# spcl/gemm_hls

Hardware: AMD Instinct MI355X
Metric: GFLOP/s, fp32 GEMM N=K=M=16384 per MI355X (tiled outer-product C=A.B), and % of fp32 MFMA peak (higher is better)
Workload: dtype f32; 1 GPU; float 16384x16384x16384 (Multiply,Add) on 1 MI355X; BASELINE configs[1]; kernel=mfma_f32_256x256x16_w8_flush4096, rows_total=16384, rows_per_gpu=16384

## Files before the change

### gemm_hls_amd/csrc/mm_mfma_f32.hip

```cpp
#include <cstdlib>
#include <type_traits>

#include "mm_common.h"

namespace mm {
namespace {

#include "mm_mfma_f32_tile.inc"
#include "mm_mfma_f32_small.inc"
#include "mm_mfma_f32_streamk.inc"

__global__ __launch_bounds__(256) void splitk_reduce_kernel(const float *__restrict__ partials, float *__restrict__ C,
                                                            size_t quads, unsigned splits) {
  const size_t i = (size_t)blockIdx.x * 256 + threadIdx.x;
  if (i >= quads) return;
  const f32x4 *src = (const f32x4 *)partials;
  f32x4 acc = src[i];
  for (unsigned s = 1; s < splits; ++s) acc += src[(size_t)s * quads + i];
  ((f32x4 *)C)[i] = acc;
}

template <typename G, bool AT = false>
int launch_geo(hipStream_t s, const Problem &p, unsigned splits = 1) {
  const unsigned tiles_n = (p.n + G::BM - 1) / G::BM, tiles_m = (p.m + G::BN - 1) / G::BN;
  static unsigned long long configured = 0;
  if (int e = ensure_dynamic_lds((const void *)mfma_f32_kernel<G, AT>, G::LDS_BYTES, configured)) return e;
  (void)hipGetLastError();
  if (splits <= 1) {
    hipLaunchKernelGGL((mfma_f32_kernel<G, AT>), dim3(tiles_n * tiles_m), dim3(G::THREADS), G::LDS_BYTES, s,
                       (const float *)p.a, (const float *)p.b, (float *)p.c, p.n, p.k, p.m, tiles_n, tiles_m,
                       band_rows(G::BM, G::BN, G::MIN_WAVES), 0u, (float *)nullptr);
    return (int)hipGetLastError();
  }
  const unsigned chunk = ((p.k + splits - 1) / splits + 31u) & ~31u;
  const size_t plane = (size_t)p.n * p.m;
  int dev = 0;
  hipError_t e = hipGetDevice(&dev);
  if (e != hipSuccess) return (int)e;
  hipMemPool_t pool = nullptr;
  if (int rc = workspace_pool(dev, &pool)) return rc;
  float *ws = nullptr;
  if ((e = hipMallocFromPoolAsync((void **)&ws, plane * splits * sizeof(float), pool, s)) != hipSuccess) return (int)e;
  hipLaunchKernelGGL((mfma_f32_kernel<G, AT>), dim3(tiles_n * tiles_m * splits), dim3(G::THREADS), G::LDS_BYTES, s,
                     (const float *)p.a, (const float *)p.b, (float *)p.c, p.n, p.k, p.m, tiles_n, tiles_m,
                     band_rows(G::BM, G::BN, G::MIN_WAVES), chunk, ws);
  int rc = (int)hipGetLastError();
  if (rc == 0) {
    const size_t quads = plane / 4;
    hipLaunchKernelGGL(splitk_reduce_kernel, dim3((unsigned)((quads + 255) / 256)), dim3(256), 0, s, ws, (float *)p.c, quads, splits);
    rc = (int)hipGetLastError();
  }
  const hipError_t f = hipFreeAsync(ws, s);
  return rc ? rc : (int)f;
}

template <typename G, bool AT, bool SEED>
__global__ __launch_bounds__(G::THREADS, G::MIN_WAVES) void mfma_f32_batched_kernel(
    const float *__restrict__ A, const float *__restrict__ B, float *__restrict__ C, unsigned N, unsigned K, unsigned M,
    unsigned tiles_n, unsigned tiles_m, unsigned kBand, unsigned batch, size_t stride_a, size_t stride_b, size_t stride_c) {
  const unsigned lin = batched_tile(A, B, C, tiles_n * tiles_m, batch, stride_a, stride_b, stride_c);
  const unsigned band = lin / (kBand * tiles_m), within = lin % (kBand * tiles_m);
  const unsigned rows_in_band = min(kBand, tiles_n - band * kBand);
  const unsigned tile_row = band * kBand + within % rows_in_band;
  const unsigned tile_col = within / rows_in_band;
  tile_body<G, AT, false, SEED>(A, B, C, N, K, M, K, M, N, M, tile_row * G::BM, tile_col * G::BN);
}

template <typename G, bool AT, bool SEED>
int launch_geo_batched_seed(hipStream_t s, const Problem &p) {
  const unsigned tiles_n = (p.n + G::BM - 1) / G::BM, tiles_m = (p.m + G::BN - 1) / G::BN;
  static unsigned long long configured = 0;
  (void)hipGetLastError();
  if (int e = ensure_dynamic_lds((const void *)mfma_f32_batched_kernel<G, AT, SEED>, G::LDS_BYTES, configured)) return e;
  hipLaunchKernelGGL((mfma_f32_batched_kernel<G, AT, SEED>), dim3(tiles_n * tiles_m * p.batch), dim3(G::THREADS), G::LDS_BYTES,
                     s, (const float *)p.a, (const float *)p.b, (float *)p.c, p.n, p.k, p.m, tiles_n, tiles_m,
                     band_rows(G::BM, G::BN, G::MIN_WAVES), p.batch, p.stride_a, p.stride_b, p.stride_c);
  return (int)hipGetLastError();
}

template <typename G, bool AT = false>
int launch_geo_batched(hipStream_t s, const Problem &p) {
  return p.seed ? launch_geo_batched_seed<G, AT, true>(s, p) : launch_geo_batched_seed<G, AT, false>(s, p);
}

using T128x256 = Geo<2, 2, 2, 16, Chain::FlushIntoC, 256, Reads::Pipelined, Dma::ScalarBase>;
using T128x256v = Geo<2, 2, 2, 16, Chain::FlushIntoC, 256, Reads::Pipelined, Dma::VectorAddress>;
using T256x256 = Geo<2, 4, 2, 16, Chain::FlushIntoC, 256, Reads::Pipelined, Dma::ScalarBase>;
using T256x256v = Geo<2, 4, 2, 16, Chain::FlushIntoC, 256, Reads::Pipelined, Dma::VectorAddress>;
using T128x128 = Geo<1, 4, 1, 32, Chain::FlushIntoC, 128, Reads::Pipelined, Dma::ScalarBase>;
using T128x128v = Geo<1, 4, 1, 32, Chain::FlushIntoC, 128, Reads::Pipelined, Dma::VectorAddress>;
using X128x256x32_2lvl = Geo<2, 2, 2, 32, Chain::TwoLevel, 16, Reads::CompilerPlaced, Dma::VectorAddress>;
using X256x256_single = Geo<2, 4, 2, 16, Chain::Single, 1, Reads::CompilerPlaced, Dma::VectorAddress>;

struct VariantInfo { int id; const char *name; unsigned bm, bn, bk, waves; };
template <typename G> constexpr VariantInfo info_of(int id, const char *name) { return {id, name, G::BM, G::BN, G::BK, G::NW}; }
constexpr VariantInfo kVariants[] = {
    info_of<T128x256>(33, "mfma_f32_128x256x16_w4x2_flush4096"),
    info_of<T256x256>(8, "mfma_f32_256x256x16_w8_flush4096"),
    info_of<T128x128>(35, "mfma_f32_128x128x32_w4x2_flush4096"),
    info_of<Small>(64, "mfma_f32_64x64x32_w4x2_flush4096"),
    info_of<X128x256x32_2lvl>(0, "mfma_f32_128x256x32_w4_2lvl"),
    info_of<X256x256_single>(3, "mfma_f32_256x256x16_w8"),
};

const VariantInfo *find_variant(int v) {
  for (const VariantInfo &i : kVariants)
    if (i.id == v) return &i;
  return nullptr;
}

}

int mfma_f32_num_variants() { return (int)(sizeof(kVariants) / sizeof(kVariants[0])); }
int mfma_f32_variant_id(int index) { return index >= 0 && index < mfma_f32_num_variants() ? kVariants[index].id : -1; }

static const TileCandidate kAutoCands[] = {{33, 128, 256, 2, 1.00}, {8, 256, 256, 1, 0.991}, {35, 128, 128, 2, 0.993}};

static bool streamk_wins(const Problem &p) {
  if (p.a_transposed || p.k % 32 != 0 || p.k < 256 || p.n_total) return false;
  if ((unsigned long long)((p.n + 127) / 128) * ((p.m + 127) / 128) * (p.k / 32) >= (1ull << 31)) return false;
  const double tiles = (double)((p.n + 127) / 128) * ((p.m + 127) / 128);
  const unsigned tn = (p.n + 127) / 128, tm = (p.m + 127) / 128;
  const bool teams_4x4 = tn % 4 == 0 && tm % 4 == 0;
  if (tiles <= 256 || tiles > (teams_4x4 ? 4096 : 2304)) return false;
  double whole = 0;
  pick_tile(kAutoCands, 3, p.n, p.m, &whole);
  const double sk = (2.0 * tiles / 512 + 0.25) * 128 * 128 / 0.993;
  return sk < 0.99 * whole;
}

template <typename G>
static int launch_small(hipStream_t s, const Problem &p, unsigned splits) {
  const unsigned tiles_n = (p.n + G::BM - 1) / G::BM, tiles_m = (p.m + G::BN - 1) / G::BN;
  static unsigned long long configured = 0;
  if (int e = ensure_dynamic_lds((const void *)mfma_f32_small_kernel<G>, G::LDS_BYTES, configured)) return e;
  (void)hipGetLastError();
  const unsigned kband = band_rows(G::BM, G::BN, G::PER_CU);
  if (splits <= 1) {
    hipLaunchKernelGGL((mfma_f32_small_kernel<G>), dim3(tiles_n * tiles_m), dim3(G::THREADS), G::LDS_BYTES, s, (const float *)p.a,
                       (const float *)p.b, (float *)p.c, p.n, p.k, p.m, tiles_n, tiles_m, kband, 0u, (float *)nullptr);
    return (int)hipGetLastError();
  }
  const unsigned chunk = ((p.k + splits - 1) / splits + 31u) & ~31u;
  if ((unsigned long long)(splits - 1) * chunk >= p.k) return kErrNotSupported;
  const size_t plane = (size_t)p.n * p.m;
  int dev = 0;
  hipError_t e = hipGetDevice(&dev);
  if (e != hipSuccess) return (int)e;
  hipMemPool_t pool = nullptr;
  if (int rc = workspace_pool(dev, &pool)) return rc;
  float *ws = nullptr;
  if ((e = hipMallocFromPoolAsync((void **)&ws, plane * splits * sizeof(float), pool, s)) != hipSuccess) return (int)e;
  hipLaunchKernelGGL((mfma_f32_small_kernel<G>), dim3(tiles_n * tiles_m * splits), dim3(G::THREADS), G::LDS_BYTES, s, (const float *)p.a,
                     (const float *)p.b, (float *)p.c, p.n, p.k, p.m, tiles_n, tiles_m, kband, chunk, ws);
  int rc = (int)hipGetLastError();
  if (rc == 0) {
    const size_t quads = plane / 4;
    hipLaunchKernelGGL(splitk_reduce_kernel, dim3((unsigned)((quads + 255) / 256)), dim3(256), 0, s, ws, (float *)p.c, quads, splits);
    rc = (int)hipGetLastError();
  }
  const hipError_t f = hipFreeAsync(ws, s);
  return rc ? rc : (int)f;
}

static unsigned auto_split_chunks(unsigned long long tiles, unsigned k) {
  unsigned s = tiles <= 192 ? (unsigned)(512 / tiles) : 1;
  if (s > 8) s = 8;
  while (s > 1 && k / s < 256) --s;
  return s;
}

static bool small_fits(const Problem &p) {
  return !p.a_transposed && 64ull * p.k * 4ull < (1ull << 32) && 32ull * p.m * 4ull < (1ull << 32);
}

static unsigned small_split_chunks(const Problem &p) {
  const unsigned rows = p.n_total ? p.n_total : p.n;
  const unsigned long long t64 = (unsigned long long)((rows + 63) / 64) * ((p.m + 63) / 64);
  if (tuning(TUNE_F32_SPLITK) == 1 || t64 > 128) return 1;
  unsigned s = (unsigned)(256 / t64);
  if (s > 8) s = 8;
  while (s > 1 && p.k / s < 512) --s;
  const double slabs = (p.k + 31) / 32;
  return (s > 1 && 13.5 + (slabs / s) * 0.52 < slabs * 0.52) ? s : 1;
}
static bool small_wins(const Problem &p) {
  if (!small_fits(p) || p.k < 32) return false;
  const unsigned rows = p.n_total ? p.n_total : p.n;
  const unsigned long long t64 = (unsigned long long)((rows + 63) / 64) * ((p.m + 63) / 64), t128 = (unsigned long long)((rows + 127) / 128) * ((p.m + 127) / 128);
  if (t64 > 512) return false;
  const double slabs = (p.k + 31) / 32;
  const unsigned ss = small_split_chunks(p);
  const double t_small = 3.5 + (ss > 1 ? 13.5 : 0.0) + (slabs / ss) * (t64 * ss <= 256 ? 0.52 : 0.90);
  const unsigned s = tuning(TUNE_F32_SPLITK) == 1 ? 1 : auto_split_chunks(t128, p.k);
  const double t_128 = (s > 1 ? 18.5 : 5.0) + (slabs / s) * (t128 * s <= 256 ? 1.79 : 3.49);
  return t_small < t_128;
}

int mfma_f32_auto_variant(const Problem &p) {
  const int knob = tuning(TUNE_F32_SPLITK);
  if (knob < 0 && streamk_wins(p)) return 35;
  const int v = pick_tile(kAutoCands, 3, p.n, p.m);
  if (v == 35 && (knob < 0 || knob == 1) && small_wins(p)) return 64;
  if (v == 33) {
    const unsigned long long t256 = (unsigned long long)((p.n + 255) / 256) * ((p.m + 255) / 256);
    if (t256 % 256 == 0 && t256 >= 4 * 256) return 8;
  }
  return v;
}

bool mfma_f32_serves(const Problem &p) {
  if (!(p.n >= 1 && p.m >= 4 && p.k >= 8 && p.m % 4 == 0 && p.k % 8 == 0)) return false;
  return !p.a_transposed || (p.n >= 4 && p.n % 4 == 0);
}

static bool transposes_first(const Problem &p, int variant_knob) {
  if (!p.a_transposed || variant_knob >= 0) return false;
  const unsigned long long tiles = (unsigned long long)((p.n + 255) / 256) * ((p.m + 255) / 256), rounds = (tiles + 255) / 256;
  if ((double)tiles >= 0.93 * (double)(rounds * 256)) return false;
  return (unsigned long long)p.n * p.k * sizeof(float) <= (2ull << 30);
}
static Problem as_row_major(const Problem &p) {
  Problem q = p;
  q.a_transposed = false;
  return q;
}

__global__ __launch_bounds__(256) void transpose_kxn_kernel(const float *__restrict__ src, float *__restrict__ dst, unsigned K, unsigned N) {
  __shared__ float tile[64][65];
  const unsigned blocks_n = (N + 63) / 64;
  const unsigned k0 = (blockIdx.x / blocks_n) * 64, n0 = (blockIdx.x % blocks_n) * 64;
#pragma unroll
  for (int i = 0; i < 4; ++i) {
    const unsigned idx = threadIdx.x + 256 * i, r = idx >> 4, c = (idx & 15u) * 4;
    if (k0 + r < K && n0 + c < N) {
      const f32x4 v = *(const f32x4 *)(src + (size_t)(k0 + r) * N + n0 + c);
#pragma unroll
      for (int j = 0; j < 4; ++j) tile[r][c + j] = v[j];
    }
  }
  __syncthreads();
#pragma unroll
  for (int i = 0; i < 4; ++i) {
    const unsigned idx = threadIdx.x + 256 * i, r = idx >> 4, c = (idx & 15u) * 4;
    if (n0 + r < N && k0 + c < K) {
      f32x4 v;
#pragma unroll
      for (int j = 0; j < 4; ++j) v[j] = tile[c + j][r];
      *(f32x4 *)(dst + (size_t)(n0 + r) * K + k0 + c) = v;
    }
  }
}

int mfma_f32_resolve(const Problem &p, int variant) {
  if (!mfma_f32_serves(p)) return -1;
  if (p.a_transposed) {
    if (transposes_first(p, variant)) return mfma_f32_resolve(as_row_major(p), variant);
    return 8;
  }
  if (variant < 0) variant = mfma_f32_auto_variant(p);
  if (variant == 64 && !small_fits(p)) return -1;
  return find_variant(variant) ? variant : -1;
}

int mfma_f32_splitk(const Problem &p, int variant) {
  if (p.a_transposed) return transposes_first(p, tuning(TUNE_F32_VARIANT)) ? mfma_f32_splitk(as_row_major(p), variant) : 1;
  if (variant == 64) {
    const int forced = tuning(TUNE_F32_SPLITK);
    unsigned s = forced >= 2 && forced <= 8 ? (unsigned)forced : tuning(TUNE_F32_VARIANT) >= 0 ? 1u : small_split_chunks(p);
    while (s > 1 && p.k / s < 64) --s;
    return (int)s;
  }
  if (variant != 35) return 1;
  const int knob = tuning(TUNE_F32_SPLITK);
  const unsigned long long sk_units = (unsigned long long)((p.n + 127) / 128) * ((p.m + 127) / 128) * (p.k / 32);
  if (knob == 0 || knob == 9 || knob == 11 || knob == 12) return (p.k % 32 == 0 && p.k >= 64 && sk_units < (1ull << 31)) ? knob : 1;
  const unsigned rows = p.n_total ? p.n_total : p.n;
  const unsigned long long tiles = (unsigned long long)((rows + 127) / 128) * ((p.m + 127) / 128);
  unsigned s;
  if (knob >= 1) s = (unsigned)knob;
  else if (tuning(TUNE_F32_VARIANT) >= 0) s = 1;
  else if (streamk_wins(p)) return 0;
  else return (int)auto_split_chunks(tiles, p.k);
  if (s > 8) s = 8;
  while (s > 1 && p.k / s < 256) --s;
  return (int)s;
}

const char *mfma_f32_name(int v) {
  const VariantInfo *i = find_variant(v);
  return i ? i->name : "?";
}

const char *mfma_f32_launch_name(const Problem &p, int v) {
  static const char *const split_names[] = {nullptr, nullptr, "mfma_f32_128x128x32_w4x2_splitk2", "mfma_f32_128x128x32_w4x2_splitk3",
                                            "mfma_f32_128x128x32_w4x2_splitk4", "mfma_f32_128x128x32_w4x2_splitk5",
                                            "mfma_f32_128x128x32_w4x2_splitk6", "mfma_f32_128x128x32_w4x2_splitk7",
                                            "mfma_f32_128x128x32_w4x2_splitk8"};
  static const char *const small_split_names[] = {nullptr, nullptr, "mfma_f32_64x64x32_w4x2_splitk2", "mfma_f32_64x64x32_w4x2_splitk3",
                                                  "mfma_f32_64x64x32_w4x2_splitk4", "mfma_f32_64x64x32_w4x2_splitk5",
                                                  "mfma_f32_64x64x32_w4x2_splitk6", "mfma_f32_64x64x32_w4x2_splitk7",
                                                  "mfma_f32_64x64x32_w4x2_splitk8"};
  const int splits = mfma_f32_splitk(p, v);
  if (v == 64 && splits > 1) return small_split_names[splits];
  if (splits == 0) return "mfma_f32_128x128x32_w4x2_streamk";
  if (splits == 9) return "mfma_f32_128x128x32_w4x2_streamk_fixup";
  if (splits == 11) return "mfma_f32_128x128x32_w4x2_streamk_two_kernels";
  if (splits == 12) return "mfma_f32_128x128x32_w4x2_streamk_ticket";
  return splits > 1 ? split_names[splits] : mfma_f32_name(v);
}

void mfma_f32_geometry(int v, unsigned *bm, unsigned *bn, unsigned *bk, unsigned *waves) {
  const VariantInfo *i = find_variant(v);
  if (!i) i = find_variant(8);
  *bm = i->bm; *bn = i->bn; *bk = i->bk; *waves = i->waves;
}

static bool sdma_fits(const Problem &p, unsigned bk) {
  const unsigned long long span = 256ull * (p.a_transposed ? 1ull : p.k) * 4ull, spanb = 32ull * (p.m > p.n ? p.m : p.n) * 4ull;
  return p.k >= bk && span < (1ull << 32) && spanb < (1ull << 32);
}

int mfma_f32_batched_resolve(const Problem &p, int variant) {
  if (!mfma_f32_serves(p)) return -1;
  if (p.a_transposed) return 8;
  if (variant == 33 || variant == 8 || variant == 35) return variant;
  return pick_tile(kAutoCands, 3, p.n, p.m, nullptr, p.batch ? p.batch : 1);
}

int launch_mfma_f32_batched(hipStream_t s, const Problem &p, int v) {
  if (!mfma_f32_serves(p)) return kErrNotSupported;
  if (p.a_transposed) return sdma_fits(p, 16) ? launch_geo_batched<T256x256, true>(s, p) : launch_geo_batched<T256x256v, true>(s, p);
  switch (v) {
    case 33: return sdma_fits(p, 16) ? launch_geo_batched<T128x256>(s, p) : launch_geo_batched<T128x256v>(s, p);
    case 8: return sdma_fits(p, 16) ? launch_geo_batched<T256x256>(s, p) : launch_geo_batched<T256x256v>(s, p);
    case 35: return sdma_fits(p, 32) ? launch_geo_batched<T128x128>(s, p) : launch_geo_batched<T128x128v>(s, p);
  }
  return kErrNotSupported;
}

int launch_mfma_f32(hipStream_t s, const Problem &p, int variant) {
  const int v = mfma_f32_resolve(p, variant);
  if (v < 0) return kErrNotSupported;
  if (p.a_transposed) {
    if (!transposes_first(p, variant)) return sdma_fits(p, 16) ? launch_geo<T256x256, true>(s, p) : launch_geo<T256x256v, true>(s, p);
    int dev = 0;
    hipError_t e = hipGetDevice(&dev);
    if (e != hipSuccess) return (int)e;
    hipMemPool_t pool = nullptr;
    if (int rc = workspace_pool(dev, &pool)) return rc;
    float *an = nullptr;
    if ((e = hipMallocFromPoolAsync((void **)&an, (size_t)p.n * p.k * sizeof(float), pool, s)) != hipSuccess) return (int)e;
    (void)hipGetLastError();
    hipLaunchKernelGGL(transpose_kxn_kernel, dim3(((p.n + 63) / 64) * ((p.k + 63) / 64)), dim3(256), 0, s, (const float *)p.a, an, p.k, p.n);
    int rc = (int)hipGetLastError();
    if (rc == 0) {
      Problem q = as_row_major(p);
      q.a = an;
      rc = launch_mfma_f32(s, q, variant);
    }
    const hipError_t f = hipFreeAsync(an, s);
    return rc ? rc : (int)f;
  }
  switch (v) {
    case 33: return sdma_fits(p, 16) ? launch_geo<T128x256>(s, p) : launch_geo<T128x256v>(s, p);
    case 8: return sdma_fits(p, 16) ? launch_geo<T256x256>(s, p) : launch_geo<T256x256v>(s, p);
    case 35: {
      const int splits = mfma_f32_splitk(p, v);
      if (splits == 0) return sdma_fits(p, 32) ? launch_streamk_arrive<T128x128>(s, p) : launch_streamk_arrive<T128x128v>(s, p);
      if (splits == 11) return sdma_fits(p, 32) ? launch_streamk_teams<T128x128>(s, p) : launch_streamk_teams<T128x128v>(s, p);
      if (splits == 12) return sdma_fits(p, 32) ? launch_streamk_arrive<T128x128, Combine::Ticket>(s, p) : launch_streamk_arrive<T128x128v, Combine::Ticket>(s, p);
      if (splits == 9) return sdma_fits(p, 32) ? launch_streamk<T128x128>(s, p) : launch_streamk<T128x128v>(s, p);
      return sdma_fits(p, 32) ? launch_geo<T128x128>(s, p, (unsigned)splits) : launch_geo<T128x128v>(s, p, (unsigned)splits);
    }
    case 64: return launch_small<Small>(s, p, (unsigned)mfma_f32_splitk(p, v));
    case 0: return launch_geo<X128x256x32_2lvl>(s, p);
    case 3: return launch_geo<X256x256_single>(s, p);
  }
  return kErrNotSupported;
}

}
```

### gemm_hls_amd/csrc/mm_mfma_f32_tile.inc

```

using f32x4 = __attribute__((ext_vector_type(4))) float;
using f32x16 = __attribute__((ext_vector_type(16))) float;
typedef const __attribute__((address_space(1))) void *gptr_t;
typedef __attribute__((address_space(3))) void *lptr_t;

enum class Chain { Single, TwoLevel, FlushIntoC };
enum class Reads { CompilerPlaced, Pipelined };
enum class Dma { VectorAddress, ScalarBase };

template <int TM_, int WM_, int WN_, int BK_, Chain CHAIN_, int CHUNK_, Reads READS_, Dma DMA_>
struct Geo {
  static constexpr Chain CHAIN = CHAIN_;
  static constexpr Reads READS = READS_;
  static constexpr Dma DMA = DMA_;
  static constexpr int CHUNK = CHUNK_;
  static constexpr int TM = TM_, WM = WM_, WN = WN_, BK = BK_, NS = 2;
  static constexpr int TN = 4;
  static constexpr int NW = WM * WN;
  static constexpr int THREADS = NW * 64;
  static constexpr int BM = WM * TM * 32, BN = WN * 128;
  static constexpr int CPR = BK / 4;
  static constexpr int SWZ_SHIFT = (CPR == 4) ? 2 : 1;
  static constexpr int A_BYTES = BM * BK * 4, B_BYTES = BK * BN * 4;
  static constexpr int STAGE_BYTES = A_BYTES + B_BYTES;
  static constexpr int LDS_BYTES = NS * STAGE_BYTES;
  static constexpr int MIN_WAVES =
      (NW == 4 && 2 * LDS_BYTES <= 160 * 1024 && (CHAIN_ == Chain::TwoLevel ? 2 : 1) * TM * TN * 16 <= 128) ? 2 : 1;
  static constexpr int NA = A_BYTES / 1024, NB = B_BYTES / 1024;
  static constexpr int LA = NA / NW, LB = NB / NW;
  static constexpr int KG = BK / 8;
  static_assert(BK == 16 || BK == 32, "BK");
  static_assert(NA % NW == 0 && NB % NW == 0, "DMA instructions must split evenly over waves");
  static_assert(LDS_BYTES <= 160 * 1024, "LDS");
  static_assert(DMA_ == Dma::VectorAddress || READS_ == Reads::Pipelined, "the scalar-base DMA pieces are placed by hand");
};

template <typename G, bool AT, bool AGENT_STORES = false, bool SEED = false>
__device__ __forceinline__ void tile_body(const float *__restrict__ A, const float *__restrict__ B, float *__restrict__ Cst,
                                          unsigned N, unsigned K, unsigned M, unsigned lda, unsigned ldc, unsigned Nst,
                                          unsigned Mst, unsigned row0, unsigned col0) {
  constexpr int TM = G::TM, TN = G::TN, BK = G::BK, NS = G::NS, CPR = G::CPR;
  constexpr bool TWO_LEVEL = G::CHAIN == Chain::TwoLevel, FLUSH = G::CHAIN == Chain::FlushIntoC;
  constexpr bool PIPELINED = G::READS == Reads::Pipelined, SDMA = G::DMA == Dma::ScalarBase;
  extern __shared__ __attribute__((aligned(16))) char smem[];
  static_assert(!AGENT_STORES || G::TM == 1, "agent-scope stores are wired into the predicated write-back only");
  auto store_quad = [](f32x4 *dst, f32x4 v) {
    if constexpr (AGENT_STORES) asm volatile("global_store_dwordx4 %0, %1, off sc1\n\ts_nop 1" ::"v"(dst), "v"(v) : "memory");
    else *dst = v;
  };

  const unsigned lane = threadIdx.x & 63u;
  const unsigned wave = __builtin_amdgcn_readfirstlane(threadIdx.x >> 6);
  const unsigned wm = wave / G::WN, wn = wave % G::WN;
  const unsigned lo = lane & 31u, hi = lane >> 5;

  size_t a_row_off[G::LA];
  unsigned a_kchunk[G::LA];
#pragma unroll
  for (int i = 0; i < G::LA; ++i) {
    const unsigned slot = (wave + G::NW * i) * 64 + lane;
    if (AT) {
      a_kchunk[i] = slot / (G::BM / 4);
      a_row_off[i] = min(row0 + (slot % (G::BM / 4)) * 4, N - 4);
    } else {
      const unsigned row = slot / CPR, pc = slot % CPR;
      a_kchunk[i] = pc ^ ((row >> G::SWZ_SHIFT) & (CPR - 1));
      a_row_off[i] = (size_t)min(row0 + row, N - 1) * lda;
    }
  }
  unsigned b_krow[G::LB];
  unsigned b_col[G::LB];
#pragma unroll
  for (int i = 0; i < G::LB; ++i) {
    const unsigned slot = (wave + G::NW * i) * 64 + lane;
    b_krow[i] = slot / (G::BN / 4);
    b_col[i] = min(col0 + (slot % (G::BN / 4)) * 4, M - 4);
  }

  auto stage = [&](unsigned buf, unsigned k0) {
    char *base = smem + buf * G::STAGE_BYTES;
#pragma unroll
    for (int i = 0; i < G::LA; ++i) {
      const float *src;
      if (AT) src = A + (size_t)min(k0 + a_kchunk[i], K - 1) * N + a_row_off[i];
      else src = A + a_row_off[i] + min(k0 + a_kchunk[i] * 4, K - 4);
      __builtin_amdgcn_global_load_lds((gptr_t)src, (lptr_t)(base + (wave + G::NW * i) * 1024), 16, 0, 0);
    }
#pragma unroll
    for (int i = 0; i < G::LB; ++i) {
      const unsigned kr = min(k0 + b_krow[i], K - 1);
      const float *src = B + (size_t)kr * M + b_col[i];
      __builtin_amdgcn_global_load_lds((gptr_t)src, (lptr_t)(base + G::A_BYTES + (wave + G::NW * i) * 1024), 16, 0, 0);
    }
  };

  unsigned voa[G::LA], vob[G::LB];
  if (SDMA) {
#pragma unroll
    for (int i = 0; i < G::LA; ++i) {
      const unsigned slot = (wave + G::NW * i) * 64 + lane, row = slot / CPR;
      if (AT) voa[i] = a_kchunk[i] * N * 4u + ((unsigned)a_row_off[i] - row0) * 4u;
      else voa[i] = (min(row0 + row, N - 1) - row0) * lda * 4u + a_kchunk[i] * 16u;
    }
#pragma unroll
    for (int i = 0; i < G::LB; ++i) vob[i] = b_krow[i] * M * 4u + (b_col[i] - col0) * 4u;
  }
  const unsigned lds_base = (unsigned)(size_t)(__attribute__((address_space(3))) char *)smem;
  auto dma_piece_s = [&](unsigned buf, unsigned k0, int i) {
    const unsigned kc = min(k0, K - BK);
    const bool is_a = i < G::LA;
    const int j = is_a ? i : i - G::LA;
    unsigned long long base = !is_a ? (unsigned long long)(B + (size_t)kc * M + col0)
                              : AT ? (unsigned long long)(A + (size_t)kc * N + row0) : (unsigned long long)(A + (size_t)row0 * lda + kc);
    const unsigned blo = __builtin_amdgcn_readfirstlane((unsigned)base), bhi = __builtin_amdgcn_readfirstlane((unsigned)(base >> 32));
    base = ((unsigned long long)bhi << 32) | blo;
    const unsigned la = lds_base + buf * G::STAGE_BYTES + (is_a ? 0 : G::A_BYTES) + (wave + G::NW * j) * 1024;
    const unsigned vo = is_a ? voa[j] : vob[j];
    unsigned keep;
    asm volatile("s_mov_b32 %0, m0\n\ts_mov_b32 m0, %3\n\ts_nop 0\n\tglobal_load_lds_dwordx4 %1, %2\n\ts_mov_b32 m0, %0"
                 : "=&s"(keep) : "v"(vo), "s"(base), "s"(la) : "memory");
  };
  auto stage_any = [&](unsigned buf, unsigned k0) {
    if constexpr (SDMA) {
#pragma unroll
      for (int i = 0; i < G::LA + G::LB; ++i) dma_piece_s(buf, k0, i);
    } else {
      stage(buf, k0);
    }
  };

  const unsigned a_swz = hi ^ ((lo >> G::SWZ_SHIFT) & (CPR - 1));
  const unsigned a_frag_base = AT ? (4 * hi) * (G::BM * 4) + (wm * TM * 32 + TM * lo) * 4
                                  : (wm * TM * 32 + lo) * (BK * 4);
  const unsigned b_frag_base = G::A_BYTES + (4 * hi) * (G::BN * 4) + (wn * 128 + 4 * lo) * 4;

  f32x16 acc[TM][TN];
#pragma unroll
  for (int mi = 0; mi < TM; ++mi)
#pragma unroll
    for (int t = 0; t < TN; ++t) acc[mi][t] = (f32x16)0.0f;
  f32x16 master[TWO_LEVEL ? TM : 1][TWO_LEVEL ? TN : 1];
  if (TWO_LEVEL) {
#pragma unroll
    for (int mi = 0; mi < TM; ++mi)
#pragma unroll
      for (int t = 0; t < TN; ++t) master[mi][t] = (f32x16)0.0f;
  }

  auto load_frags = [&](unsigned buf, int kg, f32x4 (&af)[TM], f32x4 (&bf)[4]) {
    const char *base = smem + buf * G::STAGE_BYTES;
    const unsigned achunk = ((unsigned)(2 * kg) ^ a_swz) * 16;
    if (AT) {
      using fvec = __attribute__((ext_vector_type(TM))) float;
#pragma unroll
      for (int p = 0; p < 4; ++p) {
        const fvec v = *(const fvec *)(base + a_frag_base + (kg * 8 + p) * (G::BM * 4));
#pragma unroll
        for (int mi = 0; mi < TM; ++mi) af[mi][p] = v[mi];
      }
    } else {
#pragma unroll
      for (int mi = 0; mi < TM; ++mi)
        af[mi] = *(const f32x4 *)(base + a_frag_base + mi * 32 * (BK * 4) + achunk);
    }
#pragma unroll
    for (int p = 0; p < 4; ++p)
      bf[p] = *(const f32x4 *)(base + b_frag_base + (kg * 8 + p) * (G::BN * 4));
  };

  auto mfma_group = [&](const f32x4 (&af)[TM], const f32x4 (&bf)[4]) {
#pragma unroll
    for (int p = 0; p < 4; ++p)
#pragma unroll
      for (int mi = 0; mi < TM; ++mi)
#pragma unroll
        for (int t = 0; t < TN; ++t)
          acc[mi][t] = __builtin_amdgcn_mfma_f32_32x32x2f32(af[mi][p], bf[p][t], acc[mi][t], 0, 0, 0);
  };

  typedef __attribute__((address_space(1))) f32x4 *gquad_t;
  const bool interior_block = col0 + wn * 128 + 128 <= Mst && row0 + wm * TM * 32 + TM * 32 <= Nst &&
                              (unsigned long long)(TM * 32) * ldc * 4ull < (1ull << 32);
  auto rmw_interior = [&](bool accumulate, auto batchc, auto value) {
    constexpr int BATCH = decltype(batchc)::value;
    unsigned Mv = ldc;
    asm volatile("" : "+s"(Mv));
    char *base = (char *)(Cst + (size_t)(row0 + wm * TM * 32) * Mv + col0 + wn * 128);
    const unsigned lane_off = ((AT ? TM * 4 * hi : 4 * hi) * Mv + 4 * lo) * 4u;
#pragma unroll
    for (int mi = 0; mi < TM; ++mi)
#pragma unroll
      for (int r0 = 0; r0 < 16; r0 += BATCH) {
        f32x4 old[BATCH];
#pragma unroll
        for (int j = 0; j < BATCH; ++j) {
          const int r = r0 + j, ri = (r & 3) + 8 * (r >> 2), lrow = AT ? TM * ri + mi : mi * 32 + ri;
          old[j] = accumulate ? *(gquad_t)(base + (lane_off + (unsigned)lrow * Mv * 4u)) : (f32x4)0.0f;
        }
#pragma unroll
        for (int j = 0; j < BATCH; ++j) {
          const int r = r0 + j, ri = (r & 3) + 8 * (r >> 2), lrow = AT ? TM * ri + mi : mi * 32 + ri;
          f32x4 v;
#pragma unroll
          for (int tt = 0; tt < TN; ++tt) v[tt] = value(mi, tt, r);
          *(gquad_t)(base + (lane_off + (unsigned)lrow * Mv * 4u)) = v + old[j];
        }
        __builtin_amdgcn_sched_barrier(0);
      }
  };

  auto flush_tile = [&](bool accumulate) {
    if (PIPELINED && TM >= 2 && interior_block) {
      rmw_interior(accumulate, std::integral_constant<int, 4>{}, [&](int mi, int tt, int r) { return acc[mi][tt][r]; });
#pragma unroll
      for (int mi = 0; mi < TM; ++mi)
#pragma unroll
        for (int tt = 0; tt < TN; ++tt) acc[mi][tt] = (f32x16)0.0f;
      return;
    }
    const unsigned ccol = col0 + wn * 128 + 4 * lo;
    unsigned ldv = ldc;
    asm volatile("" : "+s"(ldv));
#pragma unroll
    for (int mi = 0; mi < TM; ++mi) {
#pragma unroll
      for (int r = 0; r < 16; ++r) {
        const unsigned ri = (r & 3) + 8 * (r >> 2) + 4 * hi;
        const unsigned row = row0 + wm * TM * 32 + (AT ? TM * ri + mi : mi * 32 + ri);
        if (ccol < Mst && row < Nst) {
          f32x4 *dst = (f32x4 *)(Cst + (size_t)row * ldv + ccol);
          f32x4 v;
#pragma unroll
          for (int tt = 0; tt < TN; ++tt) v[tt] = acc[mi][tt][r];
          if (accumulate) v += *dst;
          store_quad(dst, v);
        }
      }
#pragma unroll
      for (int tt = 0; tt < TN; ++tt) acc[mi][tt] = (f32x16)0.0f;
    }
  };

  const unsigned num_tiles = (K + BK - 1) / BK;
  constexpr int L = G::LA + G::LB;

#pragma unroll
  for (int s = 0; s < NS; ++s) stage_any(s, s * BK);
  asm volatile("s_waitcnt vmcnt(%0)" ::"n"((NS - 1) * L) : "memory");
  __builtin_amdgcn_s_barrier();

  f32x4 af0[TM], bf0[4], af1[TM], bf1[4];
  load_frags(0, 0, af0, bf0);

  auto mfma_half = [&](const f32x4 (&af)[TM], const f32x4 (&bf)[4], int h) {
#pragma unroll
    for (int p = 2 * h; p < 2 * h + 2; ++p)
#pragma unroll
      for (int mi = 0; mi < TM; ++mi)
#pragma unroll
        for (int t = 0; t < TN; ++t)
          acc[mi][t] = __builtin_amdgcn_mfma_f32_32x32x2f32(af[mi][p], bf[p][t], acc[mi][t], 0, 0, 0);
  };
  auto slab = [&](unsigned t) {
    const unsigned buf = t % NS;
#pragma unroll
    for (int kg = 0; kg < G::KG; ++kg) {
      f32x4(&afc)[TM] = (kg & 1) ? af1 : af0;
      f32x4(&bfc)[4] = (kg & 1) ? bf1 : bf0;
      f32x4(&afn)[TM] = (kg & 1) ? af0 : af1;
      f32x4(&bfn)[4] = (kg & 1) ? bf0 : bf1;
      if (PIPELINED) {
        constexpr int NM = 8 * TM, NR = TM + 4;
        constexpr bool EARLY = L + NR > NM;
        static_assert(L + NR <= 2 * NM, "a k-group has too few MFMAs to spread the DMA pieces and reads over");
        __builtin_amdgcn_sched_barrier(0);
        if (kg + 1 < G::KG) {
          mfma_half(afc, bfc, 0);
          __builtin_amdgcn_sched_barrier(0);
          load_frags(buf, kg + 1, afn, bfn);
          __builtin_amdgcn_sched_barrier(0);
          mfma_half(afc, bfc, 1);
        } else {
          if (!EARLY) {
            mfma_half(afc, bfc, 0);
            __builtin_amdgcn_sched_barrier(0);
          }
          asm volatile("s_waitcnt vmcnt(%0) lgkmcnt(0)" ::"n"((NS - 2) * L) : "memory");
          __builtin_amdgcn_s_barrier();
          __builtin_amdgcn_sched_barrier(0);
          if constexpr (SDMA) {
            constexpr int TOTAL = (EARLY ? 2 : 1) * NM, P0 = EARLY ? 0 : 2;
            auto mfma_one = [&](int idx) {
              const int p = P0 + idx / (TM * TN), mi = (idx / TN) % TM, tt = idx % TN;
              acc[mi][tt] = __builtin_amdgcn_mfma_f32_32x32x2f32(afc[mi][p], bfc[p][tt], acc[mi][tt], 0, 0, 0);
            };
#pragma unroll
            for (int i = 0; i < L; ++i) {
              mfma_one(i);
              dma_piece_s(buf, (t + NS) * BK, i);
              __builtin_amdgcn_sched_barrier(0);
            }
            load_frags((t + 1) % NS, 0, afn, bfn);
#pragma unroll
            for (int i = L; i < TOTAL; ++i) mfma_one(i);
#pragma unroll
            for (int i = 0; i < NR; ++i) {
              __builtin_amdgcn_sched_group_barrier(0x008, 1, 0);
              __builtin_amdgcn_sched_group_barrier(0x100, 1, 0);
            }
            __builtin_amdgcn_sched_group_barrier(0x008, TOTAL - L - NR, 0);
            __builtin_amdgcn_sched_barrier(0);
            continue;
          }
          stage(buf, (t + NS) * BK);
          load_frags((t + 1) % NS, 0, afn, bfn);
          if (EARLY) mfma_half(afc, bfc, 0);
          mfma_half(afc, bfc, 1);
#pragma unroll
          for (int i = 0; i < L; ++i) {
            __builtin_amdgcn_sched_group_barrier(0x008, 1, 0);
            __builtin_amdgcn_sched_group_barrier(0x020, 1, 0);
          }
#pragma unroll
          for (int i = 0; i < NR; ++i) {
            __builtin_amdgcn_sched_group_barrier(0x008, 1, 0);
            __builtin_amdgcn_sched_group_barrier(0x100, 1, 0);
          }
          __builtin_amdgcn_sched_group_barrier(0x008, (EARLY ? 2 : 1) * NM - L - NR, 0);
        }
        __builtin_amdgcn_sched_barrier(0);
        continue;
      }
      if (kg + 1 < G::KG) {
        load_frags(buf, kg + 1, afn, bfn);
      } else {
        asm volatile("s_waitcnt vmcnt(%0) lgkmcnt(0)" ::"n"((NS - 2) * L) : "memory");
        __builtin_amdgcn_s_barrier();
        stage(buf, (t + NS) * BK);
        load_frags((t + 1) % NS, 0, afn, bfn);
      }
      mfma_group(afc, bfc);
    }
  };

  const unsigned steady = num_tiles - 1;
  static_assert(!SEED || FLUSH, "the seed enters through the flush into C");
  bool flushed = SEED;
  if (FLUSH) {
    for (unsigned t0 = 0; t0 < steady; t0 += G::CHUNK) {
      const unsigned tend = min(t0 + (unsigned)G::CHUNK, steady);
      for (unsigned t = t0; t < tend; ++t) slab(t);
      if (tend < steady && K > tend * BK + 32) {
        asm volatile("s_waitcnt vmcnt(0)" ::: "memory");
        flush_tile(flushed);
        asm volatile("s_waitcnt vmcnt(0)" ::: "memory");
        flushed = true;
      }
    }
  } else if (TWO_LEVEL) {
    for (unsigned t0 = 0; t0 < steady; t0 += G::CHUNK) {
      const unsigned tend = min(t0 + (unsigned)G::CHUNK, steady);
      for (unsigned t = t0; t < tend; ++t) slab(t);
#pragma unroll
      for (int mi = 0; mi < TM; ++mi)
#pragma unroll
        for (int tt = 0; tt < TN; ++tt) {
          master[mi][tt] += acc[mi][tt];
          acc[mi][tt] = (f32x16)0.0f;
        }
    }
  } else {
    for (unsigned t = 0; t < steady; ++t) slab(t);
  }

  {
    const unsigned t = num_tiles - 1;
    const int groups = (int)((K - t * BK) / 8);
    const int shift = SDMA ? G::KG - groups : 0;
    for (int kg = 0; kg < groups; ++kg) {
      load_frags(t % NS, kg + shift, af0, bf0);
      mfma_group(af0, bf0);
    }
  }

  asm volatile("s_waitcnt vmcnt(0)" ::: "memory");

  auto write_tile = [&](bool accumulate) {
    if (PIPELINED && TM >= 2 && interior_block) {
      rmw_interior(accumulate, std::integral_constant<int, (TM * TN > 8 ? 4 : 8)>{}, [&](int mi, int tt, int r) {
        float x = acc[mi][tt][r];
        if (TWO_LEVEL) x += master[mi][tt][r];
        return x;
      });
      return;
    }
    const unsigned ccol = col0 + wn * 128 + 4 * lo;
    if (ccol < Mst) {
#pragma unroll
      for (int mi = 0; mi < TM; ++mi) {
#pragma unroll
        for (int r = 0; r < 16; ++r) {
          const unsigned ri = (r & 3) + 8 * (r >> 2) + 4 * hi;
          const unsigned row = row0 + wm * TM * 32 + (AT ? TM * ri + mi : mi * 32 + ri);
          if (row < Nst) {
            f32x4 *dst = (f32x4 *)(Cst + (size_t)row * ldc + ccol);
            f32x4 v;
#pragma unroll
            for (int tt = 0; tt < TN; ++tt) {
              float x = acc[mi][tt][r];
              if (TWO_LEVEL) x += master[mi][tt][r];
              v[tt] = x;
            }
            if (accumulate) v += *dst;
            store_quad(dst, v);
          }
        }
      }
    }
  };
  if (FLUSH && flushed) write_tile(true); else write_tile(false);
}

template <typename G, bool AT>
__global__ __launch_bounds__(G::THREADS, G::MIN_WAVES) void mfma_f32_kernel(const float *__restrict__ A,
                                                              const float *__restrict__ B,
                                                              float *__restrict__ C, unsigned N,
                                                              unsigned K, unsigned M,
                                                              unsigned tiles_n, unsigned tiles_m,
                                                              unsigned kBand, unsigned kChunk, float *__restrict__ partials) {
  const unsigned nwg = tiles_n * tiles_m;
  const unsigned lda = K;
  unsigned bid = blockIdx.x;
  if (kChunk) {
    const unsigned split = bid / nwg;
    bid -= split * nwg;
    const unsigned kbeg = split * kChunk;
    A += AT ? (size_t)kbeg * N : (size_t)kbeg;
    B += (size_t)kbeg * M;
    C = partials + (size_t)split * N * M;
    K = min(kChunk, K - kbeg);
  }
  const unsigned lin = xcd_remap(bid, nwg);
  const unsigned band = lin / (kBand * tiles_m), within = lin % (kBand * tiles_m);
  const unsigned rows_in_band = min(kBand, tiles_n - band * kBand);
  const unsigned tile_row = band * kBand + within % rows_in_band;
  const unsigned tile_col = within / rows_in_band;
  tile_body<G, AT>(A, B, C, N, K, M, lda, M, N, M, tile_row * G::BM, tile_col * G::BN);
}
```

Before: 150,700 GFLOP/s.

## Keep part of the flushed accumulator partials on chip in LDS and registers

Adds KEEP_LDS/KEEP_REG parameters so that, at each periodic flush into C, some of each wave's accumulator blocks go to a per-wave LDS slot (3 blocks) or spare registers (1 block) instead of a global read-modify-write. The 256x256 variants now keep 4 of their 8 blocks on chip, which removes part of the C traffic at every flush and the reload of those partials. In exchange it uses 96KB more LDS, more registers, and a per-component store path for partially kept quads. That path may produce narrower, less efficient global accesses.

```diff
diff --git a/gemm_hls_amd/csrc/mm_mfma_f32.hip b/gemm_hls_amd/csrc/mm_mfma_f32.hip
--- a/gemm_hls_amd/csrc/mm_mfma_f32.hip
+++ b/gemm_hls_amd/csrc/mm_mfma_f32.hip
@@ -85,8 +85,8 @@
 
 using T128x256 = Geo<2, 2, 2, 16, Chain::FlushIntoC, 256, Reads::Pipelined, Dma::ScalarBase>;
 using T128x256v = Geo<2, 2, 2, 16, Chain::FlushIntoC, 256, Reads::Pipelined, Dma::VectorAddress>;
-using T256x256 = Geo<2, 4, 2, 16, Chain::FlushIntoC, 256, Reads::Pipelined, Dma::ScalarBase>;
-using T256x256v = Geo<2, 4, 2, 16, Chain::FlushIntoC, 256, Reads::Pipelined, Dma::VectorAddress>;
+using T256x256 = Geo<2, 4, 2, 16, Chain::FlushIntoC, 256, Reads::Pipelined, Dma::ScalarBase, 3, 1>;
+using T256x256v = Geo<2, 4, 2, 16, Chain::FlushIntoC, 256, Reads::Pipelined, Dma::VectorAddress, 3, 1>;
 using T128x128 = Geo<1, 4, 1, 32, Chain::FlushIntoC, 128, Reads::Pipelined, Dma::ScalarBase>;
 using T128x128v = Geo<1, 4, 1, 32, Chain::FlushIntoC, 128, Reads::Pipelined, Dma::VectorAddress>;
 using X128x256x32_2lvl = Geo<2, 2, 2, 32, Chain::TwoLevel, 16, Reads::CompilerPlaced, Dma::VectorAddress>;
diff --git a/gemm_hls_amd/csrc/mm_mfma_f32_tile.inc b/gemm_hls_amd/csrc/mm_mfma_f32_tile.inc
--- a/gemm_hls_amd/csrc/mm_mfma_f32_tile.inc
+++ b/gemm_hls_amd/csrc/mm_mfma_f32_tile.inc
@@ -8,7 +8,7 @@
 enum class Reads { CompilerPlaced, Pipelined };
 enum class Dma { VectorAddress, ScalarBase };
 
-template <int TM_, int WM_, int WN_, int BK_, Chain CHAIN_, int CHUNK_, Reads READS_, Dma DMA_>
+template <int TM_, int WM_, int WN_, int BK_, Chain CHAIN_, int CHUNK_, Reads READS_, Dma DMA_, int KEEP_LDS_ = 0, int KEEP_REG_ = 0>
 struct Geo {
   static constexpr Chain CHAIN = CHAIN_;
   static constexpr Reads READS = READS_;
@@ -23,7 +23,9 @@
   static constexpr int SWZ_SHIFT = (CPR == 4) ? 2 : 1;
   static constexpr int A_BYTES = BM * BK * 4, B_BYTES = BK * BN * 4;
   static constexpr int STAGE_BYTES = A_BYTES + B_BYTES;
-  static constexpr int LDS_BYTES = NS * STAGE_BYTES;
+  static constexpr int KEEP_LDS = KEEP_LDS_, KEEP_REG = KEEP_REG_;
+  static constexpr int RING_BYTES = NS * STAGE_BYTES;
+  static constexpr int LDS_BYTES = RING_BYTES + NW * KEEP_LDS * 4096;
   static constexpr int MIN_WAVES =
       (NW == 4 && 2 * LDS_BYTES <= 160 * 1024 && (CHAIN_ == Chain::TwoLevel ? 2 : 1) * TM * TN * 16 <= 128) ? 2 : 1;
   static constexpr int NA = A_BYTES / 1024, NB = B_BYTES / 1024;
@@ -32,6 +34,8 @@
   static_assert(BK == 16 || BK == 32, "BK");
   static_assert(NA % NW == 0 && NB % NW == 0, "DMA instructions must split evenly over waves");
   static_assert(LDS_BYTES <= 160 * 1024, "LDS");
+  static_assert(KEEP_LDS_ >= 0 && KEEP_REG_ >= 0 && KEEP_LDS_ + KEEP_REG_ <= TM_ * 4, "kept blocks");
+  static_assert(KEEP_LDS_ + KEEP_REG_ == 0 || CHAIN_ == Chain::FlushIntoC, "only the chain flush into C has partials to keep");
   static_assert(DMA_ == Dma::VectorAddress || READS_ == Reads::Pipelined, "the scalar-base DMA pieces are placed by hand");
 };
 
@@ -147,6 +151,39 @@
       for (int t = 0; t < TN; ++t) master[mi][t] = (f32x16)0.0f;
   }
 
+  constexpr int KL = FLUSH ? G::KEEP_LDS : 0, KR = FLUSH ? G::KEEP_REG : 0, KEPT = KL + KR;
+  f32x16 keepr[KR ? KR : 1];
+  auto kept_get = [&](int b) {
+    if (b >= KL) return keepr[b - KL];
+    const char *slot = smem + G::RING_BYTES + (wave * KL + b) * 4096 + lane * 16;
+    f32x16 v;
+#pragma unroll
+    for (int q = 0; q < 4; ++q) {
+      const f32x4 x = *(const f32x4 *)(slot + q * 1024);
+#pragma unroll
+      for (int j = 0; j < 4; ++j) v[4 * q + j] = x[j];
+    }
+    return v;
+  };
+  auto kept_put = [&](int b, f32x16 v) {
+    if (b >= KL) {
+      keepr[b - KL] = v;
+      return;
+    }
+    char *slot = smem + G::RING_BYTES + (wave * KL + b) * 4096 + lane * 16;
+#pragma unroll
+    for (int q = 0; q < 4; ++q) {
+      f32x4 x;
+#pragma unroll
+      for (int j = 0; j < 4; ++j) x[j] = v[4 * q + j];
+      *(f32x4 *)(slot + q * 1024) = x;
+    }
+  };
+  auto c_from = [](int mi, int first) {
+    const int c = first - mi * TN;
+    return c < 0 ? 0 : c > TN ? TN : c;
+  };
+
   auto load_frags = [&](unsigned buf, int kg, f32x4 (&af)[TM], f32x4 (&bf)[4]) {
     const char *base = smem + buf * G::STAGE_BYTES;
     const unsigned achunk = ((unsigned)(2 * kg) ^ a_swz) * 16;
@@ -179,23 +216,44 @@
   };
 
   typedef __attribute__((address_space(1))) f32x4 *gquad_t;
+  typedef __attribute__((address_space(1))) float *gfloat_t;
+  auto load_comps = [](char *p, int from) {
+    if (from == 0) return *(gquad_t)p;
+    f32x4 v = (f32x4)0.0f;
+#pragma unroll
+    for (int c = 1; c < 4; ++c)
+      if (c >= from) v[c] = *(gfloat_t)(p + 4 * c);
+    return v;
+  };
+  auto store_comps = [](char *p, f32x4 v, int from) {
+    if (from == 0) {
+      *(gquad_t)p = v;
+      return;
+    }
+#pragma unroll
+    for (int c = 1; c < 4; ++c)
+      if (c >= from) *(gfloat_t)(p + 4 * c) = v[c];
+  };
   const bool interior_block = col0 + wn * 128 + 128 <= Mst && row0 + wm * TM * 32 + TM * 32 <= Nst &&
                               (unsigned long long)(TM * 32) * ldc * 4ull < (1ull << 32);
-  auto rmw_interior = [&](bool accumulate, auto batchc, auto value) {
-    constexpr int BATCH = decltype(batchc)::value;
+  auto rmw_interior = [&](bool accumulate, auto batchc, auto firstc, auto storeallc, auto value) {
+    constexpr int BATCH = decltype(batchc)::value, FIRST_C = decltype(firstc)::value;
+    constexpr bool STORE_ALL = decltype(storeallc)::value;
     unsigned Mv = ldc;
     asm volatile("" : "+s"(Mv));
     char *base = (char *)(Cst + (size_t)(row0 + wm * TM * 32) * Mv + col0 + wn * 128);
     const unsigned lane_off = ((AT ? TM * 4 * hi : 4 * hi) * Mv + 4 * lo) * 4u;
 #pragma unroll
-    for (int mi = 0; mi < TM; ++mi)
+    for (int mi = 0; mi < TM; ++mi) {
+      const int from = c_from(mi, FIRST_C);
+      if (from == TN && !STORE_ALL) continue;
 #pragma unroll
       for (int r0 = 0; r0 < 16; r0 += BATCH) {
         f32x4 old[BATCH];
 #pragma unroll
         for (int j = 0; j < BATCH; ++j) {
           const int r = r0 + j, ri = (r & 3) + 8 * (r >> 2), lrow = AT ? TM * ri + mi : mi * 32 + ri;
-          old[j] = accumulate ? *(gquad_t)(base + (lane_off + (unsigned)lrow * Mv * 4u)) : (f32x4)0.0f;
+          old[j] = accumulate ? load_comps(base + (lane_off + (unsigned)lrow * Mv * 4u), from) : (f32x4)0.0f;
         }
 #pragma unroll
         for (int j = 0; j < BATCH; ++j) {
@@ -203,15 +261,43 @@
           f32x4 v;
 #pragma unroll
           for (int tt = 0; tt < TN; ++tt) v[tt] = value(mi, tt, r);
-          *(gquad_t)(base + (lane_off + (unsigned)lrow * Mv * 4u)) = v + old[j];
+          f32x4 sum = v + old[j];
+#pragma unroll
+          for (int tt = 0; tt < TN; ++tt)
+            if (tt < from) sum[tt] = v[tt];
+          store_comps(base + (lane_off + (unsigned)lrow * Mv * 4u), sum, STORE_ALL ? 0 : from);
         }
         __builtin_amdgcn_sched_barrier(0);
       }
+    }
+  };
+
+  auto load_c_block = [&](int mi, int tt) {
+    f32x16 v;
+    const unsigned ccol = col0 + wn * 128 + 4 * lo;
+#pragma unroll
+    for (int r = 0; r < 16; ++r) {
+      const unsigned ri = (r & 3) + 8 * (r >> 2) + 4 * hi;
+      const unsigned row = row0 + wm * TM * 32 + (AT ? TM * ri + mi : mi * 32 + ri);
+      v[r] = (ccol < Mst && row < Nst) ? Cst[(size_t)row * ldc + ccol + tt] : 0.0f;
+    }
+    return v;
+  };
+  auto flush_kept = [&](bool first) {
+#pragma unroll
+    for (int b = 0; b < KEPT; ++b) {
+      const int mi = b / TN, tt = b % TN;
+      f32x16 sum = acc[mi][tt];
+      if (!first) sum += kept_get(b);
+      kept_put(b, sum);
+      acc[mi][tt] = (f32x16)0.0f;
+    }
   };
 
   auto flush_tile = [&](bool accumulate) {
     if (PIPELINED && TM >= 2 && interior_block) {
-      rmw_interior(accumulate, std::integral_constant<int, 4>{}, [&](int mi, int tt, int r) { return acc[mi][tt][r]; });
+      rmw_interior(accumulate, std::integral_constant<int, 4>{}, std::integral_constant<int, KEPT>{}, std::false_type{},
+                   [&](int mi, int tt, int r) { return acc[mi][tt][r]; });
 #pragma unroll
       for (int mi = 0; mi < TM; ++mi)
 #pragma unroll
@@ -229,11 +315,21 @@
         const unsigned row = row0 + wm * TM * 32 + (AT ? TM * ri + mi : mi * 32 + ri);
         if (ccol < Mst && row < Nst) {
           f32x4 *dst = (f32x4 *)(Cst + (size_t)row * ldv + ccol);
-          f32x4 v;
-#pragma unroll
-          for (int tt = 0; tt < TN; ++tt) v[tt] = acc[mi][tt][r];
-          if (accumulate) v += *dst;
-          store_quad(dst, v);
+          if (c_from(mi, KEPT) == 0) {
+            f32x4 v;
+#pragma unroll
+            for (int tt = 0; tt < TN; ++tt) v[tt] = acc[mi][tt][r];
+            if (accumulate) v += *dst;
+            store_quad(dst, v);
+          } else {
+#pragma unroll
+            for (int tt = 0; tt < TN; ++tt)
+              if (tt >= c_from(mi, KEPT)) {
+                float x = acc[mi][tt][r];
+                if (accumulate) x += ((float *)dst)[tt];
+                ((float *)dst)[tt] = x;
+              }
+          }
         }
       }
 #pragma unroll
@@ -243,6 +339,15 @@
 
   const unsigned num_tiles = (K + BK - 1) / BK;
   constexpr int L = G::LA + G::LB;
+
+  bool onchip = false;
+  if constexpr (SEED && KEPT > 0) {
+#pragma unroll
+    for (int b = 0; b < KEPT; ++b) kept_put(b, load_c_block(b / TN, b % TN));
+    onchip = true;
+    asm volatile("s_waitcnt vmcnt(0)" ::: "memory");
+    __builtin_amdgcn_sched_barrier(0);
+  }
 
 #pragma unroll
   for (int s = 0; s < NS; ++s) stage_any(s, s * BK);
@@ -352,9 +457,10 @@
       for (unsigned t = t0; t < tend; ++t) slab(t);
       if (tend < steady && K > tend * BK + 32) {
         asm volatile("s_waitcnt vmcnt(0)" ::: "memory");
+        if constexpr (KEPT > 0) flush_kept(!onchip);
         flush_tile(flushed);
         asm volatile("s_waitcnt vmcnt(0)" ::: "memory");
-        flushed = true;
+        flushed = onchip = true;
       }
     }
   } else if (TWO_LEVEL) {
@@ -385,9 +491,10 @@
 
   asm volatile("s_waitcnt vmcnt(0)" ::: "memory");
 
-  auto write_tile = [&](bool accumulate) {
+  auto write_tile = [&](bool accumulate, auto firstc) {
+    constexpr int FIRST_C = decltype(firstc)::value;
     if (PIPELINED && TM >= 2 && interior_block) {
-      rmw_interior(accumulate, std::integral_constant<int, (TM * TN > 8 ? 4 : 8)>{}, [&](int mi, int tt, int r) {
+      rmw_interior(accumulate, std::integral_constant<int, (TM * TN > 8 ? 4 : 8)>{}, firstc, std::true_type{}, [&](int mi, int tt, int r) {
         float x = acc[mi][tt][r];
         if (TWO_LEVEL) x += master[mi][tt][r];
         return x;
@@ -411,14 +518,29 @@
               if (TWO_LEVEL) x += master[mi][tt][r];
               v[tt] = x;
             }
-            if (accumulate) v += *dst;
+            if (c_from(mi, FIRST_C) == 0) {
+              if (accumulate) v += *dst;
+            } else {
+#pragma unroll
+              for (int tt = 0; tt < TN; ++tt)
+                if (accumulate && tt >= c_from(mi, FIRST_C)) v[tt] += ((const float *)dst)[tt];
+            }
             store_quad(dst, v);
           }
         }
       }
     }
   };
-  if (FLUSH && flushed) write_tile(true); else write_tile(false);
+  constexpr std::integral_constant<int, 0> all_in_c{};
+  if constexpr (KEPT > 0) {
+    if (onchip) {
+#pragma unroll
+      for (int b = 0; b < KEPT; ++b) acc[b / TN][b % TN] += kept_get(b);
+      write_tile(true, std::integral_constant<int, KEPT>{});
+      return;
+    }
+  }
+  if (FLUSH && flushed) write_tile(true, all_in_c); else write_tile(false, all_in_c);
 }
 
 template <typename G, bool AT>
```

Measured after the change: 151,000 GFLOP/s (median of 6 runs). No clear change (+0.2%).
